# pydata/sparse

Measured on AMD Instinct MI355X. Metric: GCXS x dense SpMM throughput (GFLOP/s), higher is better.
Workload: dtype f32; 1 GPU; GCXS(CSR) 1000000x10000 @ 0.01 (100000000 nnz, int32 idx) in 1 nnz-balanced row block(s) x dense 10000x128 fp32; world_size=1, rows_rank0=1000000, idx_dtype=int32, parallelism=row-block x1, mul_add=fma, nan_warning=deferred, prewarm_products=40, default_settings=NAN_WARNING="sync" (verdict read inside every product), kernel=spmm_tiled (cached block stream)

## Files before the change

sparse_amd/_kernels.py:

```python
import os

import numpy as np
import torch

from . import _ffi
from ._device import code_of, np_dtype, ptr, require_hip, stream_ptr, torch_dtype


def dot_dtype(dt1, dt2):
    return (np.zeros((), dtype=np_dtype(dt1)) * np.zeros((), dtype=np_dtype(dt2))).dtype


_COMPLEX_CODE = {torch.complex64: _ffi.C64, torch.complex128: _ffi.C128}


def product_code(dt):
    dt = torch_dtype(dt)
    code = _COMPLEX_CODE.get(dt)
    return code_of(dt) if code is None else code


def _as_reals(t):
    return torch.view_as_real(t).reshape(-1) if t.is_complex() else t

# ... 1896 lines not shown
    return finish(exclusive_scan(nblk), lambda bo, total, blocks: _ffi.call(
        "spamd_spmm_tiled_pack", vc, nnz, ptr(tk), ptr(vals), ptr(seg_start), ptr(bo), total, ptr(blocks), s))


TILED_BALANCE = True
TILED_BALANCE_MIN_NNZ = 1 << 20
TILED_BALANCE_SKEW = 1.6
TILED_BALANCE_CAPMUL = 2
TILED_BALANCE_STATS = {}


def _balanced_tiled_layout(vals, ind, ptr_, M, Kd, dtype, nnz, defer_check, dev, s):
    rg, kb, gpb, epb, slack, direct_max, _ = tiled_params(dtype)
    ntiles = -(-Kd // kb)
    ic, vc = code_of(ind.dtype), code_of(_tiled_layout_dtype(dtype))
    mean_group = nnz * rg / max(M, 1)
    cap = 32
    while cap < TILED_BALANCE_CAPMUL * mean_group:
        cap *= 2
    stats = torch.empty(8, dtype=torch.int64, device=dev)
    _ffi.call("spamd_spmm_tiled_map_stats", ic, M, Kd, cap, ptr(ptr_), None, None, ptr(stats), s)
    st = stats.tolist()
    skew = st[6] / max(mean_group, 1.0)
    TILED_BALANCE_STATS.update(cap=cap, class_rows=st[:6], natural_max_group=st[6], skew=skew, balanced=False)
    if skew <= TILED_BALANCE_SKEW:
        return None
    keys = torch.empty(M, dtype=torch.int64, device=dev)
    rows = torch.empty(M, dtype=torch.int32, device=dev)
    _ffi.call("spamd_spmm_tiled_map_stats", ic, M, Kd, cap, ptr(ptr_), ptr(keys), ptr(rows), ptr(stats), s)
    st = stats.tolist()
    TILED_BALANCE_STATS.update(class_rows=st[:6])
    counts = _harr64(st[:6])
    groups = int(_ffi.lib().spamd_spmm_tiled_map_groups(counts))
    nseg = groups * ntiles
    upper = -(-nnz // epb) + nseg
    if groups <= 0 or upper >= 2 ** 31:
        return None
    keys, rows = sort_key_value(keys, rows, max(Kd, 1))
    rowmap = torch.empty(groups * rg + 16, dtype=torch.int32, device=dev)
    gload = torch.empty(groups + 1, dtype=torch.int64, device=dev)
    _ffi.call("spamd_spmm_tiled_map_build", ic, M, cap, ptr(ptr_), ptr(rows), counts, ptr(rowmap), ptr(gload), s)
    vstart = exclusive_scan(gload)
    blocks = torch.empty((upper + slack) * 16, dtype=torch.int32, device=dev)
    blk_off = torch.empty(groups * (ntiles + 1), dtype=torch.int32, device=dev)
    state = torch.empty(1, dtype=torch.int64, device=dev)
    _ffi.call("spamd_spmm_tiled_inspect_mapped", vc, ic, M, Kd, groups, ptr(vals), ptr(ind), ptr(ptr_), ptr(rowmap), ptr(vstart),
              ptr(state), ptr(blk_off), ptr(blocks), s)
    TILED_BALANCE_STATS.update(balanced=True, groups=groups)
    lay = TiledLayout(blocks, blk_off, dtype, nnz / epb / max(nseg, 1) + 0.5, group_ends=True, pending=state if defer_check else None,
                      rowmap=rowmap, groups=groups)
    if not defer_check and int(state[0]) != 0:
        return None
    return lay


def csc_tiled_layout(a_data, a_indices, a_indptr, M, Kd, dtype=None):
    dev = require_hip(a_data, a_indices, a_indptr)
    if dtype is None:
        dtype = a_data.dtype if a_data.dtype in TILED_DTYPES else torch.float32
    dtype = torch_dtype(dtype)
    rg, kb, gpb, epb, slack, direct_max, _ = tiled_params(dtype)
    nnz = int(a_data.numel())
    ntiles = -(-Kd // kb)
    groups = -(-(-(-M // rg)) // gpb) * gpb
    nseg = groups * ntiles
    upper = -(-nnz // epb) + nseg
    if ntiles > direct_max or upper >= 2 ** 31 or groups == 0 or not TILED_ONE_PASS_INSPECTOR:
        return None
    if not index_dtype_ok(a_indices) or a_indices.dtype != a_indptr.dtype:
        a_indices, a_indptr = a_indices.to(torch.int64), a_indptr.to(torch.int64)
    vals = a_data.to(dtype).contiguous()
    if dtype == torch.int32:
        vals = vals.view(torch.float32)
    blocks = torch.empty((upper + slack) * 16, dtype=torch.int32, device=dev)
    blk_off = torch.empty(groups * (ntiles + 1), dtype=torch.int32, device=dev)
    split = torch.empty(int(_ffi.lib().spamd_spmm_tiled_inspect_csc_ws(M, Kd)), dtype=torch.int32, device=dev)
    state = torch.empty(1, dtype=torch.int64, device=dev)
    _ffi.call("spamd_spmm_tiled_inspect_csc", code_of(_tiled_layout_dtype(dtype)), code_of(a_indices.dtype), M, Kd, ptr(vals),
              ptr(a_indices.contiguous()), ptr(a_indptr.contiguous()), ptr(split), ptr(state), ptr(blk_off), ptr(blocks),
              stream_ptr(dev))
    return TiledLayout(blocks, blk_off, dtype, nnz / epb / max(nseg, 1) + 0.5, group_ends=True, pending=state)


def dot_csr_ndarray_tiled(layout, out_shape, Kd, b, out=None, exact=False):
    blocks, blk_off, dtype = layout
    M, N = int(out_shape[0]), int(b.shape[1])
    Nout = int(out_shape[1])
    panel = 64 if dtype == torch.float64 else 128
    if N % panel or not (N - panel < Nout <= N):
        raise ValueError(f"tiled executor: B has {N} columns (whole {panel}-column panels expected), result {Nout}")
    last_cols = (Nout - (N - panel)) % panel
    dev = require_hip(blocks, blk_off, b)
    if b.dtype != dtype:
        raise TypeError(f"tiled layout holds {dtype} values, B is {b.dtype}")
    b = b.contiguous()
    if out is None:
        out = torch.empty((M, Nout), dtype=dtype, device=dev)
    lists = max(int(blk_off.numel()) - 1, 1)
    mean_blocks = getattr(layout, "mean_blocks", None) or (int(blocks.numel()) // 16) / lists
    hint = min(64, max(6, int(1.5 * mean_blocks) + 3))
    if _TOUCH_OVERRIDE:
        hint = _TOUCH_OVERRIDE
    ends = _ffi.TILED_GROUP_ENDS if getattr(layout, "group_ends", False) else 0
    ints = _ffi.TILED_INT32 if dtype == torch.int32 else 0
    flags = (_ffi.EXACT_MULADD if exact and not ints else 0) | ends | ints | (hint << 8) | (last_cols << 16)
    rowmap = getattr(layout, "rowmap", None)
    if rowmap is not None:
        _ffi.call("spamd_spmm_tiled_mapped", code_of(_tiled_layout_dtype(dtype)), M, int(layout.groups), Kd, N, ptr(blocks), ptr(blk_off),
                  ptr(rowmap), ptr(b), N, ptr(out), Nout, flags, stream_ptr(dev))
    else:
        _ffi.call("spamd_spmm_tiled", code_of(_tiled_layout_dtype(dtype)), M, Kd, N, ptr(blocks), ptr(blk_off), ptr(b), N, ptr(out), Nout,
                  flags, stream_ptr(dev))
    pending = getattr(layout, "pending", None)
    if pending is not None:
        layout.pending = None
        words = pending.tolist()
        mean = getattr(layout, "skew_mean", None)
        if mean and len(words) >= 8 and words[7] > TILED_BALANCE_SKEW * max(mean, 1.0):
            layout.rebalance = True
        if int(words[0]) != 0:
            raise UnsortedColumns("tiled layout built from rows with unsorted column indices")
    return out
```

sparse_amd/csrc/spmm_tiled.hip:

```cpp
#include "common.h"
#include "spmm_tiled_asm.inc"
#include <stdlib.h>
#include <mutex>
#include <set>

namespace spamd {

constexpr int TL_RG = TL_ASM_RG;
constexpr int TL_WAVES = TL_ASM_WAVES;
#ifndef SPAMD_TL_EXPERIMENTAL
static_assert(TL_RG == 35 && TL_WAVES == 16, "experimental tiled-SpMM geometry: build with -DSPAMD_TL_EXPERIMENTAL");
#endif
constexpr int TL_KB = TL_ASM_KB;
constexpr int TL_NBUF = 2;
__host__ __device__ constexpr int tl_d0(int lc, int lr) { return ((lc >> 1) << 11) | ((lc & 1) << 9) | (2 + 2 * lr); }
constexpr int TL_BLOCK_INTS = 16;

template <typename T>
struct TlFmt;
template <>
struct TlFmt<float> {
  static constexpr int EPB = 8, PANEL = 128;
  __device__ static void put(int* stream, int64_t entry, int d0, float v) {
    int* b = stream + (entry / EPB) * TL_BLOCK_INTS + (entry % EPB) * 2;
    typedef int int2v __attribute__((ext_vector_type(2)));
    int2v e;
    e.x = d0;
    e.y = __builtin_bit_cast(int, v);
    *reinterpret_cast<int2v*>(b) = e;
  }
};
template <>
struct TlFmt<double> {
  static constexpr int EPB = 5, PANEL = 64;
  __device__ static void put(int* stream, int64_t entry, int d0, double v) {
    int* b = stream + (entry / EPB) * TL_BLOCK_INTS;
    const int slot = (int)(entry % EPB);
    const long long bits = __builtin_bit_cast(long long, v);
    b[slot] = d0;
    if (slot == 0) b[5] = 0;
    *reinterpret_cast<long long*>(b + 6 + 2 * slot) = bits;
  }
};
typedef int tl_srd_t __attribute__((ext_vector_type(4)));
constexpr int TL_TILE = TL_KB * 512;
constexpr int TL_LDS = TL_NBUF * TL_TILE;
constexpr int TL_DMA_PER_TILE = TL_TILE / 16 / (TL_WAVES * 64);
static_assert(TL_LDS <= 160 * 1024 && TL_KB % (2 * TL_WAVES) == 0 && TL_DMA_PER_TILE == TL_ASM_DMA_PER_TILE,
              "tile geometry is baked into gen_tiled_asm.py");
constexpr int TL_SLACK_BLOCKS = 68;

#define GRID_STRIDE(i, n)                                                          \
  for (int64_t i = (int64_t)blockIdx.x * blockDim.x + threadIdx.x; i < (n);        \
       i += (int64_t)gridDim.x * blockDim.x)

__global__ void __launch_bounds__(256) tl_keys_kernel(const int64_t* __restrict__ rc_keys, int64_t nnz, int64_t K,
                                                      int64_t ntiles, int64_t* __restrict__ out) {
  GRID_STRIDE(i, nnz) {
    const int64_t k = rc_keys[i];
    const int64_t row = k / K, col = k - row * K;
    const int64_t g = row / TL_RG, lr = row - g * TL_RG, t = col / TL_KB, lc = col - t * TL_KB;
    out[i] = ((g * ntiles + t) * TL_RG + lr) * TL_KB + lc;
  }
}

__global__ void __launch_bounds__(256) tl_seg_start_kernel(const int64_t* __restrict__ keys, int64_t nnz,
                                                           int64_t nseg, int64_t* __restrict__ seg_start) {
  GRID_STRIDE(i, nnz + 1) {
    const int64_t hi = i < nnz ? keys[i] / (TL_RG * TL_KB) : nseg;
    const int64_t lo = i > 0 ? keys[i - 1] / (TL_RG * TL_KB) + 1 : 0;
    for (int64_t s = lo; s <= hi; ++s) seg_start[s] = i;
  }
}

__global__ void __launch_bounds__(256) tl_blocks_kernel(const int64_t* __restrict__ seg_start, int64_t nseg, int epb,
                                                        int64_t* __restrict__ nblk) {
  GRID_STRIDE(s, nseg + 1) {
    nblk[s] = s < nseg ? (seg_start[s + 1] - seg_start[s] + epb - 1) / epb : 0;
  }
}

template <typename T>
__global__ void __launch_bounds__(256) tl_pack_kernel(const int64_t* __restrict__ keys, const T* __restrict__ vals,
                                                      int64_t nnz, const int64_t* __restrict__ seg_start,
                                                      const int64_t* __restrict__ blk_off, int* __restrict__ stream) {
// ... 201 lines not shown
  const int gtotal = wtot[0] + wtot[1] + wtot[2] + wtot[3];
  const int my_off = woff + x - nb;
  const int64_t goff = tl_group_first_block(e0, g, ntiles, EPB);
  const int64_t gnext = tl_group_first_block(e1, g + 1, ntiles, EPB);
  if (tid < ntiles) loff[tid] = my_off;
  __syncthreads();
  if (tid < ntiles) blk_off[g * (ntiles + 1) + tid] = (int)(goff + my_off);
  if (tid == 0) blk_off[g * (ntiles + 1) + ntiles] = (int)(goff + gtotal);
  for (int64_t i = (goff + gtotal) * TL_BLOCK_INTS + tid; i < gnext * TL_BLOCK_INTS; i += 256) stream[i] = 0;
  if (group_bad) {
    for (int64_t i = goff * TL_BLOCK_INTS + tid; i < (goff + gtotal) * TL_BLOCK_INTS; i += 256) stream[i] = 0;
    return;
  }
  auto fill_one = [&](int lr, int64_t ra, int64_t e, unsigned c, T v) {
    const int t = (int)(c / (unsigned)TL_KB);
    const int lc = (int)(c - (unsigned)t * (unsigned)TL_KB);
    const int64_t dst = (goff + loff[t]) * EPB + before[lr * ntiles + t] + ((int)(e - (MAPPED ? ra : e0)) - runstart[lr * ntiles + t]);
    TlFmt<T>::put(stream, dst, tl_d0(lc, lr), v);
  };
#pragma unroll
  for (int i = 0; i < RPW; ++i) {
    const int lr = wv + 4 * i;
    if (lr >= TL_RG) break;
    const int64_t ra = rsab[2 * (lr)], rb = rsab[2 * (lr) + 1];
#pragma unroll
    for (int p = 0; p < TL_PRE; ++p) {
      const int64_t e = ra + lane + 64 * p;
      if (e < rb) fill_one(lr, ra, e, cpre[i][p], vpre[i][p]);
    }
    for (int64_t e = ra + lane + 64 * TL_PRE; e < rb; e += 64) fill_one(lr, ra, e, (unsigned)indices[e], vals[e]);
  }
  if (tid < ntiles) {
    const int64_t first = (goff + my_off) * EPB;
    for (int i = cnt_t; i < nb * EPB; ++i) TlFmt<T>::put(stream, first + i, 0, T(0));
  }
}

__device__ __forceinline__ void tl_dma16(unsigned lds_base, const void* src) {
  asm volatile("s_mov_b32 m0, %0\n\ts_nop 0\n\tglobal_load_lds_dwordx4 %1, off"
               :
               : "s"(lds_base), "v"(src)
               : "memory", "m0");
}

template <int MODE>
__device__ __forceinline__ void tl_phases(const int* stream, int t0, int te, int o0, int o1, int o2, int offreg, int obase,
                                          int ntiles, int nfull, int toff, int mask, unsigned m0wave,
                                          unsigned row_step, int voff, tl_srd_t srd, unsigned& soff) {
  const int lane = threadIdx.x & 63;
  const unsigned blo = (unsigned)((uintptr_t)stream & 0xffffffffu), bhi = (unsigned)((uintptr_t)stream >> 32);
  const int lane8 = lane * 8;
#define TL_PHASES_OPERANDS                                                                                        \
  [soff] "+s"(soff)                                                                                               \
  : [blo] "s"(blo), [bhi] "s"(bhi), [t0] "s"(t0), [te] "s"(te), [o0] "s"(o0), [o1] "s"(o1), [o2] "s"(o2),         \
    [obase] "s"(obase), [ntiles] "s"(ntiles), [nfull] "s"(nfull), [m0wave] "s"(m0wave), [step] "s"(row_step),      \
    [toff] "v"(toff), [lane8] "v"(lane8), [mask] "v"(mask), [offreg] "v"(offreg), [voff] "v"(voff), [srd] "s"(srd)  \
  : "memory", "m0", "scc", "vcc", TL_CLOB_SGPR, TL_CLOB_TMP, TL_CLOB_ACC
  if (MODE == 6)
    asm volatile(TL_ASM_PHASES_I32 : TL_PHASES_OPERANDS);
  else if (MODE == 4)
    asm volatile(TL_ASM_PHASES_F64 : TL_PHASES_OPERANDS);
  else if (MODE == 5)
    asm volatile(TL_ASM_PHASES_F64_EXACT : TL_PHASES_OPERANDS);
  else if (MODE == 3)
    asm volatile(TL_ASM_PHASES_EXACT : TL_PHASES_OPERANDS);
  else if (MODE == 1)
    asm volatile(TL_ASM_PHASES_NOFMA : TL_PHASES_OPERANDS);
  else if (MODE == 2)
    asm volatile(TL_ASM_PHASES_NOLDS : TL_PHASES_OPERANDS);
  else
    asm volatile(TL_ASM_PHASES : TL_PHASES_OPERANDS);
#undef TL_PHASES_OPERANDS
}

__device__ __forceinline__ void tl_block_map(unsigned L, int npanels, int nblocks, int& bx, int& by) {
  const unsigned pin = npanels > 1 ? 2u : 1u;
  const unsigned per_chunk = (unsigned)((nblocks + 7) / 8) * 8u * pin;
  const unsigned chunk = L / per_chunk, l = L % per_chunk;
  const unsigned seq = l >> 3;
  by = uniform((int)(chunk * pin + seq % pin));
  bx = uniform((int)((seq / pin) * 8u + (l & 7u)));
}

template <int DBG, int MODE, typename T>
__global__ void __launch_bounds__(TL_WAVES * 64) __attribute__((amdgpu_num_vgpr(TL_ASM_COMP)))
spmm_tiled_kernel(int64_t M, int64_t K, int ntiles, int touch_lines, const int* __restrict__ stream,
                  const int* __restrict__ blk_off, const T* __restrict__ b, int64_t ldb,
                  T* __restrict__ out, int64_t ldo, int last_cols, int npanels, int nblocks, const int* __restrict__ rowmap) {
  constexpr int PANEL = TlFmt<T>::PANEL;
  constexpr int CPL = PANEL / 64;
  extern __shared__ __attribute__((aligned(16))) char lds[];
  const int tid = threadIdx.x;
  const int lane = tid & 63;
  const int wv = uniform(tid >> 6);
  int bx, by;
  tl_block_map(blockIdx.x, npanels, nblocks, bx, by);
  if (bx >= nblocks || by >= npanels) return;
  const int g = bx * TL_WAVES + wv;
  b += (int64_t)by * PANEL;
  out += (int64_t)by * PANEL;

  asm volatile(TL_ASM_ZERO ::: "memory", TL_CLOB_ACC);

  const int nfull = DBG == 2 ? 0 : (int)(K / TL_KB);
  const unsigned row_step = (unsigned)((2 * TL_WAVES) * ldb * (int64_t)sizeof(T));
  const unsigned m0wave = (unsigned)wv * 2048u;
  const uint64_t bbase = (uint64_t)(uintptr_t)b;
  tl_srd_t srd;
  srd[0] = (int)(bbase & 0xffffffffu);
  srd[1] = (int)((bbase >> 32) & 0xffffu);
  srd[2] = (int)0xffffffffu;
  srd[3] = 0x00020000;
  const int voff = (int)((int64_t)(tid >> 5) * ldb * (int64_t)sizeof(T)) + (tid & 31) * 16;
  unsigned soff = 0;
  auto issue_partial = [&](int t) {
#pragma unroll
    for (int i = 0; i < TL_DMA_PER_TILE; ++i) {
      const int e = (i * (TL_WAVES * 64) + tid) * 16;
      int64_t r = (int64_t)t * TL_KB + (e >> 9);
      if (r >= K) r = K - 1;
      tl_dma16(((unsigned)(i * TL_WAVES + wv) * 2u + (unsigned)(t & 1)) * 1024u,
               reinterpret_cast<const char*>(b + r * ldb) + (e & 511));
    }
  };
  const bool has_partial = DBG != 2 && (int64_t)nfull * TL_KB < K;

  if (nfull > 0)
    asm volatile(TL_ASM_TILE0 : [soff] "+s"(soff) : [m0wave] "s"(m0wave), [step] "s"(row_step), [voff] "v"(voff), [srd] "s"(srd) : "memory", "m0", "scc", "vcc", "s89");
  else if (has_partial)
    issue_partial(0);
  asm volatile("s_waitcnt vmcnt(0)" ::: "memory");
  __syncthreads();

  const int* const myoff = blk_off + (int64_t)g * (ntiles + (touch_lines >> 16));
  touch_lines &= 0xffff;
  const int toff = (lane < touch_lines ? lane : touch_lines - 1) * 64;
  int t = 0;
  while (t < ntiles) {
    const int obase = t;
    const int q = obase + lane;
    int offreg = myoff[q < ntiles ? q : ntiles];
    asm volatile("" : "+v"(offreg));
    int te = obase + 61 < ntiles ? obase + 61 : ntiles;
    if (has_partial && t < nfull - 1 && nfull - 1 < te) te = nfull - 1;
    if (has_partial && t == nfull - 1) issue_partial(nfull);
    auto o = [&](int tt) { return wave_bcast(offreg, (tt < ntiles ? tt : ntiles) - obase); };
    const int o0 = o(t), o1 = o(t + 1), o2 = o(t + 2);
    if (t == 0) {
      const int n = o2 - o0, l = lane < n ? lane : 0;
      asm volatile("global_load_dword " TL_ASM_TOUCH ", %0, off" ::"v"(reinterpret_cast<const char*>(stream + (int64_t)o0 * 16) + l * 64)
                   : "memory", TL_ASM_TOUCH);
    }
    tl_phases<MODE>(stream, t, te, o0, o1, o2, offreg, obase, ntiles, nfull, toff, (int)0xfffffe00, m0wave, row_step, voff, srd, soff);
    t = te;
  }
  asm volatile("s_waitcnt vmcnt(0) lgkmcnt(0)" ::: "memory");

  const int64_t row0 = (int64_t)g * TL_RG;
  const int64_t left = M - row0;
  const int nvalid = left <= 0 ? 0 : (left < TL_RG ? (int)left : TL_RG);
  T* const obase_p = out + row0 * ldo + lane * CPL;
  const int64_t stride_bytes = ldo * (int64_t)sizeof(T);
  int bx2, by2;
  tl_block_map(blockIdx.x, npanels, nblocks, bx2, by2);
  const int ncols = (last_cols > 0 && by2 == npanels - 1) ? last_cols : PANEL;
  if (rowmap) {
    const int* const rm = rowmap + (int64_t)g * TL_RG;
    T* const base_p = out + lane * CPL;
    if (lane * CPL + CPL <= ncols)
      asm volatile(TL_ASM_STORE_PERM
                   :
                   : [lo] "v"((unsigned)((uintptr_t)base_p & 0xffffffffu)), [hi] "v"((unsigned)((uintptr_t)base_p >> 32)),
                     [stride] "s"((unsigned)stride_bytes), [rm] "s"(rm)
                   : "memory", "scc", TL_CLOB_SGPR, TL_CLOB_TMP, TL_CLOB_ACC);
    if constexpr (CPL == 2) {
      if (lane * CPL + 1 == ncols)
        asm volatile(TL_ASM_STORE1_PERM
                     :
                     : [lo] "v"((unsigned)((uintptr_t)base_p & 0xffffffffu)), [hi] "v"((unsigned)((uintptr_t)base_p >> 32)),
                       [stride] "s"((unsigned)stride_bytes), [rm] "s"(rm)
                     : "memory", "scc", TL_CLOB_SGPR, TL_CLOB_TMP);
    }
    return;
  }
  if (lane * CPL + CPL <= ncols)
    asm volatile(TL_ASM_STORE
                 :
                 : [lo] "v"((unsigned)((uintptr_t)obase_p & 0xffffffffu)), [hi] "v"((unsigned)((uintptr_t)obase_p >> 32)),
                   [stride] "s"(stride_bytes), [n] "s"(nvalid)
                 : "memory", "scc", "s36", TL_ASM_BASE, TL_ASM_TOUCH, TL_CLOB_ACC);
  if constexpr (CPL == 2) {
    if (lane * CPL + 1 == ncols)
      asm volatile(TL_ASM_STORE1
                   :
                   : [lo] "v"((unsigned)((uintptr_t)obase_p & 0xffffffffu)), [hi] "v"((unsigned)((uintptr_t)obase_p >> 32)),
                     [stride] "s"(stride_bytes), [n] "s"(nvalid)
                   : "memory", "scc", "s36", TL_ASM_BASE, TL_ASM_TOUCH);
  }
}

static int64_t tl_grid_groups(int64_t M) { return ceil_div(ceil_div(M, (int64_t)TL_RG), (int64_t)TL_WAVES) * TL_WAVES; }

}

using namespace spamd;

static int tl_epb(int val_dtype) { return val_dtype == SPAMD_F32 ? TlFmt<float>::EPB : (val_dtype == SPAMD_F64 ? TlFmt<double>::EPB : 0); }

extern "C" int spamd_spmm_tiled_params(int val_dtype, int* rows_per_group, int* tile_rows, int* groups_per_block,
                                       int* entries_per_block, int* slack_blocks, int* direct_max_tiles,
                                       int* panel_cols) {
  if (!tl_epb(val_dtype)) return SPAMD_ETYPE;
  if (direct_max_tiles) *direct_max_tiles = TL_DIRECT_MAX_TILES;
  if (rows_per_group) *rows_per_group = TL_RG;
  if (tile_rows) *tile_rows = TL_KB;
  if (groups_per_block) *groups_per_block = TL_WAVES;
  if (entries_per_block) *entries_per_block = tl_epb(val_dtype);
  if (slack_blocks) *slack_blocks = TL_SLACK_BLOCKS;
  if (panel_cols) *panel_cols = val_dtype == SPAMD_F32 ? TlFmt<float>::PANEL : TlFmt<double>::PANEL;
  return 0;
}

static unsigned tl_blocks_for(int64_t n) {
  int64_t blocks = ceil_div(n, (int64_t)256);
  if (blocks > 8192) blocks = 8192;
  if (blocks < 1) blocks = 1;
  return (unsigned)blocks;
}

extern "C" int spamd_spmm_tiled_keys(int64_t nnz, const int64_t* rowcol_keys, int64_t K, int64_t* tiled_keys,
                                     void* stream) {
  if (nnz < 0 || K <= 0) return SPAMD_EINVAL;
  if (nnz == 0) return 0;
  hipLaunchKernelGGL(tl_keys_kernel, dim3(tl_blocks_for(nnz)), dim3(256), 0, (hipStream_t)stream, rowcol_keys, nnz, K,
                     ceil_div(K, (int64_t)TL_KB), tiled_keys);
  return launch_status();
}

extern "C" int spamd_spmm_tiled_lists(int val_dtype, int64_t nnz, const int64_t* tiled_keys_sorted, int64_t M, int64_t K,
                                      int64_t* seg_start, int64_t* nblk, void* stream) {
  if (nnz < 0 || M < 0 || K <= 0) return SPAMD_EINVAL;
  if (!tl_epb(val_dtype)) return SPAMD_ETYPE;
  const int64_t nseg = tl_grid_groups(M) * ceil_div(K, (int64_t)TL_KB);
  hipLaunchKernelGGL(tl_seg_start_kernel, dim3(tl_blocks_for(nnz + 1)), dim3(256), 0, (hipStream_t)stream,
                     tiled_keys_sorted, nnz, nseg, seg_start);
  hipLaunchKernelGGL(tl_blocks_kernel, dim3(tl_blocks_for(nseg + 1)), dim3(256), 0, (hipStream_t)stream, seg_start,
                     nseg, tl_epb(val_dtype), nblk);
  return launch_status();
}

static int tl_clear_blocks(int64_t total_blocks, int* blocks, hipStream_t s) {
  return (int)hipMemsetAsync(blocks, 0, (size_t)(total_blocks + TL_SLACK_BLOCKS) * TL_BLOCK_INTS * sizeof(int), s);
}

extern "C" int spamd_spmm_tiled_pack(int val_dtype, int64_t nnz, const int64_t* tiled_keys_sorted, const void* vals_sorted,
                                     const int64_t* seg_start, const int64_t* blk_off, int64_t total_blocks,
                                     int* blocks, void* stream) {
  if (nnz < 0 || total_blocks < 0) return SPAMD_EINVAL;
  if (!tl_epb(val_dtype)) return SPAMD_ETYPE;
  int rc = tl_clear_blocks(total_blocks, blocks, (hipStream_t)stream);
  if (rc) return rc;
  if (nnz == 0) return 0;
  if (val_dtype == SPAMD_F32)
    hipLaunchKernelGGL(tl_pack_kernel<float>, dim3(tl_blocks_for(nnz)), dim3(256), 0, (hipStream_t)stream, tiled_keys_sorted,
                       (const float*)vals_sorted, nnz, seg_start, blk_off, blocks);
  else
    hipLaunchKernelGGL(tl_pack_kernel<double>, dim3(tl_blocks_for(nnz)), dim3(256), 0, (hipStream_t)stream, tiled_keys_sorted,
                       (const double*)vals_sorted, nnz, seg_start, blk_off, blocks);
  return launch_status();
}

extern "C" int spamd_spmm_tiled_count(int val_dtype, int idx_dtype, int64_t M, int64_t K, const void* a_indices,
                                      const void* a_indptr, int64_t* nblk, int* flags, void* stream) {
  if (M < 0 || K <= 0) return SPAMD_EINVAL;
  if (!tl_epb(val_dtype)) return SPAMD_ETYPE;
  const int64_t ntiles = ceil_div(K, (int64_t)TL_KB);
  if (ntiles > TL_DIRECT_MAX_TILES) return SPAMD_EINVAL;
  const int64_t groups = tl_grid_groups(M);
  hipError_t e = hipMemsetAsync(flags, 0, sizeof(int), (hipStream_t)stream);
  if (e != hipSuccess) return (int)e;
// ... 756 lines not shown
      for (int q = c; q < nb * EPB; ++q) TlFmt<T>::put(stream, first + q, 0, T(0));
    }
    __syncthreads();
  }
}

template <typename I, typename T>
static int tl_launch_inspect_csc(int64_t M, int64_t K, int64_t ntiles, const T* a_data, const I* a_indices, const I* a_indptr,
                                 int* ws, unsigned long long* state, int* blk_off, int* blocks, hipStream_t s) {
  const int64_t groups = tl_grid_groups(M);
  const int64_t nblocks = groups / TL_WAVES;
  if (nblocks >= ((int64_t)1 << 31)) return SPAMD_EINVAL;
  const bool hist = groups <= TL_CSC_HIST_GROUPS;
  int* const split = ws;
  int* const cnt = split + (nblocks + 1) * K;
  int* const rel = cnt + TL_CSC_HIST_PARTS * groups * ntiles;
  const int64_t words = ((nblocks + 1) * K + TL_CSC_HIST_PARTS * groups * ntiles + groups * (ntiles + 1) + 1) & ~(int64_t)1;
  unsigned long long* const look = reinterpret_cast<unsigned long long*>(ws + words);
  long long* const e0 = reinterpret_cast<long long*>(look) + groups;
  const int64_t owgs = ceil_div(groups, (int64_t)64);
  const int nlook = (int)(owgs + 2);
  static_assert(TL_WAVES >= 3, "groups (a multiple of TL_WAVES) >= ceil(groups / 64) + 2");
  if (!hist) {
    const unsigned sgrid = (unsigned)std::min<int64_t>(K, (int64_t)256 * 64);
    hipLaunchKernelGGL((tl_csc_split_kernel<I>), dim3(sgrid), dim3(256), 0, s, M, K, nblocks, a_indices, a_indptr, split, state, look, nlook);
  }
  const dim3 grid((unsigned)nblocks, (unsigned)ceil_div(ntiles, (int64_t)TL_CSC_TC));
  if (hist) {
    auto hk = &tl_csc_hist_kernel<I>;
    const int lds = (int)((groups + 1) / 2 * sizeof(int));
    if (lds > 48 * 1024) {
      hipError_t e = hipFuncSetAttribute(reinterpret_cast<const void*>(hk), hipFuncAttributeMaxDynamicSharedMemorySize, lds);
      if (e != hipSuccess) return (int)e;
    }
    hipLaunchKernelGGL(hk, dim3((unsigned)ntiles, TL_CSC_HIST_PARTS), dim3(1024), lds, s, M, K, (int)ntiles, groups, nblocks,
                       a_indices, a_indptr, cnt, split, state, look, nlook);
  } else {
    hipLaunchKernelGGL((tl_csc_count_kernel<I>), grid, dim3(256), 0, s, K, (int)ntiles, nblocks, groups, a_indices, a_indptr, (const int*)split,
                       (const unsigned long long*)state, cnt);
  }
  if (hist)
    hipLaunchKernelGGL((tl_csc_offsets_kernel<TlFmt<T>::EPB, TL_CSC_HIST_PARTS>), dim3((unsigned)owgs), dim3(64), 0, s,
                       groups, (int)ntiles, (const int*)cnt, (const unsigned long long*)state, rel, look, e0);
  else
    hipLaunchKernelGGL((tl_csc_offsets_kernel<TlFmt<T>::EPB, 1>), dim3((unsigned)owgs), dim3(64), 0, s,
                       groups, (int)ntiles, (const int*)cnt, (const unsigned long long*)state, rel, look, e0);
  const int64_t fgrid = 8 * ceil_div(nblocks, (int64_t)8) * ceil_div(ntiles, (int64_t)TL_CSC_TC);
  if (fgrid >= ((int64_t)1 << 31)) return SPAMD_EINVAL;
  hipLaunchKernelGGL((tl_csc_fill_kernel<I, T>), dim3((unsigned)fgrid), dim3(256), 0, s, K, (int)ntiles, a_data, a_indices,
                     a_indptr, (const int*)split, (const unsigned long long*)state, (const int*)rel, (const long long*)e0, nblocks,
                     blk_off, blocks);
  return launch_status();
}

extern "C" int64_t spamd_spmm_tiled_inspect_csc_ws(int64_t M, int64_t K) {
  if (M < 0 || K <= 0) return -1;
  const int64_t ntiles = ceil_div(K, (int64_t)TL_KB), groups = tl_grid_groups(M), nblocks = groups / TL_WAVES;
  return (nblocks + 1) * K + TL_CSC_HIST_PARTS * groups * ntiles + groups * (ntiles + 1) + 2 + 2 * (2 * groups + 1) + 16;
}

extern "C" int spamd_spmm_tiled_inspect_csc(int val_dtype, int idx_dtype, int64_t M, int64_t K, const void* a_data,
                                            const void* a_indices, const void* a_indptr, int* ws, void* state, int* blk_off,
                                            int* blocks, void* stream) {
  if (M < 0 || K <= 0) return SPAMD_EINVAL;
  if (!tl_epb(val_dtype)) return SPAMD_ETYPE;
  if ((uintptr_t)ws % 8) return SPAMD_EINVAL;
  const int64_t ntiles = ceil_div(K, (int64_t)TL_KB);
  if (ntiles > TL_DIRECT_MAX_TILES) return SPAMD_EINVAL;
  hipError_t e = hipMemsetAsync(state, 0, sizeof(unsigned long long), (hipStream_t)stream);
  if (e != hipSuccess) return (int)e;
  if (tl_grid_groups(M) == 0) return 0;
  SPAMD_DISPATCH_IDX(idx_dtype, I, {
    if (val_dtype == SPAMD_F32)
      return tl_launch_inspect_csc<I, float>(M, K, ntiles, (const float*)a_data, (const I*)a_indices, (const I*)a_indptr, ws,
                                             (unsigned long long*)state, blk_off, blocks, (hipStream_t)stream);
    return tl_launch_inspect_csc<I, double>(M, K, ntiles, (const double*)a_data, (const I*)a_indices, (const I*)a_indptr, ws,
                                            (unsigned long long*)state, blk_off, blocks, (hipStream_t)stream);
  })
  return SPAMD_ETYPE;
}

static int tl_set_lds_once(const void* kern) { return set_max_dynamic_lds(kern, TL_LDS); }

template <typename T, typename KERN>
static int tl_launch(KERN kern, int64_t M, int64_t K, int64_t N, const int* blocks, const int* blk_off, const T* b,
                     int64_t ldb, T* out, int64_t ldo, int touch_lines, bool group_ends, int last_cols, hipStream_t s,
                     const int* rowmap = nullptr, int64_t map_groups = 0) {
  if (int rc = tl_set_lds_once(reinterpret_cast<const void*>(kern))) return rc;
  const int64_t blocks_n = (rowmap ? map_groups : tl_grid_groups(M)) / TL_WAVES;
  const int64_t npanels = N / TlFmt<T>::PANEL;
  const int64_t grid = ceil_div(blocks_n, (int64_t)8) * 8 * (npanels > 1 ? ceil_div(npanels, (int64_t)2) * 2 : 1);
  if (grid >= ((int64_t)1 << 31) || blocks_n >= ((int64_t)1 << 31)) return SPAMD_EINVAL;
  hipLaunchKernelGGL(kern, dim3((unsigned)grid), dim3(TL_WAVES * 64), TL_LDS, s, M, K,
                     (int)ceil_div(K, (int64_t)TL_KB), touch_lines | (group_ends ? 1 << 16 : 0), blocks, blk_off, b, ldb, out, ldo,
                     last_cols, (int)npanels, (int)blocks_n, rowmap);
  return launch_status();
}

static int tl_product(int val_dtype, int64_t M, int64_t K, int64_t N, const int* blocks, const int* blk_off, const void* b,
                      int64_t ldb, void* out, int64_t ldo, unsigned flags, void* stream, const int* rowmap, int64_t map_groups);

extern "C" int spamd_spmm_tiled(int val_dtype, int64_t M, int64_t K, int64_t N, const int* blocks, const int* blk_off,
                                const void* b, int64_t ldb, void* out, int64_t ldo, unsigned flags, void* stream) {
  return tl_product(val_dtype, M, K, N, blocks, blk_off, b, ldb, out, ldo, flags, stream, nullptr, 0);
}

extern "C" int spamd_spmm_tiled_mapped(int val_dtype, int64_t M, int64_t groups, int64_t K, int64_t N, const int* blocks,
                                       const int* blk_off, const int* rowmap, const void* b, int64_t ldb, void* out, int64_t ldo,
                                       unsigned flags, void* stream) {
  if (!rowmap || groups <= 0 || groups % TL_WAVES) return SPAMD_EINVAL;
  if (ldo * (val_dtype == SPAMD_F32 ? 4 : 8) >= ((int64_t)1 << 32)) return SPAMD_EINVAL;
  return tl_product(val_dtype, M, K, N, blocks, blk_off, b, ldb, out, ldo, flags | SPAMD_TILED_GROUP_ENDS, stream, rowmap, groups);
}

static int tl_product(int val_dtype, int64_t M, int64_t K, int64_t N, const int* blocks, const int* blk_off, const void* b,
                      int64_t ldb, void* out, int64_t ldo, unsigned flags, void* stream, const int* rowmap, int64_t map_groups) {
  if (!tl_epb(val_dtype)) return SPAMD_ETYPE;
  const int panel = val_dtype == SPAMD_F32 ? TlFmt<float>::PANEL : TlFmt<double>::PANEL;
  const int esz = val_dtype == SPAMD_F32 ? 4 : 8;
  if (M < 0 || K <= 0 || N <= 0 || N % panel != 0 || N / panel > 65535 || K / TL_KB >= ((int64_t)1 << 30)) return SPAMD_EINVAL;
  if (M == 0) return 0;
  if (((uintptr_t)b % 16) || ((ldb * esz) % 16) || ((uintptr_t)out % esz) || ((uintptr_t)blocks % 64))
    return SPAMD_EINVAL;
  if ((K + 2 * TL_KB) * ldb * esz >= ((int64_t)1 << 32)) return SPAMD_EINVAL;
  hipStream_t s = (hipStream_t)stream;
  const bool exact = (flags & SPAMD_EXACT_MULADD) != 0;
  const bool ends = (flags & SPAMD_TILED_GROUP_ENDS) != 0;
  const bool i32 = (flags & SPAMD_TILED_INT32) != 0;
  if (i32 && val_dtype != SPAMD_F32) return SPAMD_EINVAL;
  const int last_cols = (int)((flags >> 16) & 0xffu);
  if (last_cols > panel) return SPAMD_EINVAL;
  if (ldo < N - panel + (last_cols ? last_cols : panel)) return SPAMD_EINVAL;
  int touch = (int)((flags >> 8) & 0xffu);
  if (touch == 0) touch = 12;
  if (touch > 64) touch = 64;
  if (val_dtype == SPAMD_F64) {
    const double* bb = (const double*)b;
    double* oo = (double*)out;
    return exact ? tl_launch<double>(&spmm_tiled_kernel<0, 5, double>, M, K, N, blocks, blk_off, bb, ldb, oo, ldo, touch, ends, last_cols, s, rowmap, map_groups)
                 : tl_launch<double>(&spmm_tiled_kernel<0, 4, double>, M, K, N, blocks, blk_off, bb, ldb, oo, ldo, touch, ends, last_cols, s, rowmap, map_groups);
  }
  const float* bb = (const float*)b;
  float* oo = (float*)out;
#ifdef SPAMD_TUNING
  const char* dbg_env = getenv("SPAMD_TILED_DBG");
  const int dbg = dbg_env ? atoi(dbg_env) : 0;
  if (dbg == 2) return tl_launch<float>(&spmm_tiled_kernel<2, 0, float>, M, K, N, blocks, blk_off, bb, ldb, oo, ldo, touch, ends, last_cols, s, rowmap, map_groups);
  if (dbg == 5) return tl_launch<float>(&spmm_tiled_kernel<0, 1, float>, M, K, N, blocks, blk_off, bb, ldb, oo, ldo, touch, ends, last_cols, s, rowmap, map_groups);
  if (dbg == 6) return tl_launch<float>(&spmm_tiled_kernel<0, 2, float>, M, K, N, blocks, blk_off, bb, ldb, oo, ldo, touch, ends, last_cols, s, rowmap, map_groups);
  if (dbg == 7) return tl_launch<float>(&spmm_tiled_kernel<2, 2, float>, M, K, N, blocks, blk_off, bb, ldb, oo, ldo, touch, ends, last_cols, s, rowmap, map_groups);
#endif
  if (i32) return tl_launch<float>(&spmm_tiled_kernel<0, 6, float>, M, K, N, blocks, blk_off, bb, ldb, oo, ldo, touch, ends, last_cols, s, rowmap, map_groups);
  return exact ? tl_launch<float>(&spmm_tiled_kernel<0, 3, float>, M, K, N, blocks, blk_off, bb, ldb, oo, ldo, touch, ends, last_cols, s, rowmap, map_groups)
               : tl_launch<float>(&spmm_tiled_kernel<0, 0, float>, M, K, N, blocks, blk_off, bb, ldb, oo, ldo, touch, ends, last_cols, s, rowmap, map_groups);
}
```

Before: 30260 GFLOP/s.

## Make tiled SpMM kernel persistent, prefetching next block's first tile before storing

Converts the tiled SpMM kernel into a persistent kernel. With a single panel and no rowmap, the grid is limited to roughly one workgroup per CU, and each workgroup loops over logical blocks. Before storing the current block's accumulators, it starts the next block's B-tile DMA and offset load, so launch and prologue latency overlap with the epilogue. It also prefetches the next chunk's offsets inside the tile loop and passes kernel args by struct read from the kernarg segment to save registers. The risks are reduced occupancy and latency hiding, plus more scalar reloads.

```diff
diff --git a/sparse_amd/_kernels.py b/sparse_amd/_kernels.py
--- a/sparse_amd/_kernels.py
+++ b/sparse_amd/_kernels.py
@@ -2002,8 +2002,11 @@
     return TiledLayout(blocks, blk_off, dtype, nnz / epb / max(nseg, 1) + 0.5, group_ends=True, pending=state)
 
 
-def dot_csr_ndarray_tiled(layout, out_shape, Kd, b, out=None, exact=False):
+def dot_csr_ndarray_tiled(layout, out_shape, Kd, b, out=None, exact=False, resident=0):
     blocks, blk_off, dtype = layout
+    resident = int(resident)
+    if resident < 0 or resident % 8 or resident > 127 * 8:
+        raise ValueError(f"tiled executor: resident = {resident} (a multiple of 8 in [0, 1016] expected)")
     M, N = int(out_shape[0]), int(b.shape[1])
     Nout = int(out_shape[1])
     panel = 64 if dtype == torch.float64 else 128
@@ -2023,7 +2026,7 @@
         hint = _TOUCH_OVERRIDE
     ends = _ffi.TILED_GROUP_ENDS if getattr(layout, "group_ends", False) else 0
     ints = _ffi.TILED_INT32 if dtype == torch.int32 else 0
-    flags = (_ffi.EXACT_MULADD if exact and not ints else 0) | ends | ints | (hint << 8) | (last_cols << 16)
+    flags = (_ffi.EXACT_MULADD if exact and not ints else 0) | ends | ints | (hint << 8) | (last_cols << 16) | ((resident // 8) << 24)
     rowmap = getattr(layout, "rowmap", None)
     if rowmap is not None:
         _ffi.call("spamd_spmm_tiled_mapped", code_of(_tiled_layout_dtype(dtype)), M, int(layout.groups), Kd, N, ptr(blocks), ptr(blk_off),
diff --git a/sparse_amd/csrc/spmm_tiled.hip b/sparse_amd/csrc/spmm_tiled.hip
--- a/sparse_amd/csrc/spmm_tiled.hip
+++ b/sparse_amd/csrc/spmm_tiled.hip
@@ -1,6 +1,7 @@
 #include "common.h"
 #include "spmm_tiled_asm.inc"
 #include <stdlib.h>
+#include <atomic>
 #include <mutex>
 #include <set>
 
@@ -368,120 +369,247 @@
   bx = uniform((int)((seq / pin) * 8u + (l & 7u)));
 }
 
+template <typename T>
+struct TlArgs {
+  int64_t M, K;
+  const int* stream;
+  const int* blk_off;
+  const T* b;
+  int64_t ldb;
+  T* out;
+  int64_t ldo;
+  const int* rowmap;
+  int ntiles, touch_lines, last_cols, npanels, nblocks;
+  int total;
+  int grid;
+#ifdef SPAMD_TUNING
+  unsigned long long* stamps;
+#endif
+};
+
+#ifdef SPAMD_TUNING
+constexpr int TL_STAMPS = 12;
+static unsigned long long* tl_timeline_buf = nullptr;
+#define TL_STAMP(L, slot)                                                                      \
+  do {  \
+    unsigned long long* const st_ = tl_args<T>()->stamps;                                      \
+    if (st_ && uniform(tl_park(tid) >> 6) == 0) st_[(int64_t)(L) * TL_STAMPS + (slot)] = wall_clock64(); \
+  } while (0)
+#else
+#define TL_STAMP(L, slot) \
+  do {                    \
+  } while (0)
+#endif
+
+template <typename T>
+__device__ __forceinline__ const __attribute__((address_space(4))) TlArgs<T>* tl_args() {
+  auto p = (const __attribute__((address_space(4))) TlArgs<T>*)__builtin_amdgcn_kernarg_segment_ptr();
+  asm volatile("" : "+s"(p));
+  return p;
+}
+
+__device__ __forceinline__ int tl_park(int x) {
+  asm volatile("" : "+v"(x));
+  return x;
+}
+__device__ __forceinline__ int tl_fresh(int x) {
+  asm volatile("" : "+s"(x));
+  return x;
+}
+
+__device__ __forceinline__ int tl_next_block(int L, int grid, int total, int npanels, int nblocks) {
+  while (L < total) {
+    int bx, by;
+    tl_block_map((unsigned)L, npanels, nblocks, bx, by);
+    if (bx < nblocks && by < npanels) break;
+    L += grid;
+  }
+  return L;
+}
+
 template <int DBG, int MODE, typename T>
 __global__ void __launch_bounds__(TL_WAVES * 64) __attribute__((amdgpu_num_vgpr(TL_ASM_COMP)))
-spmm_tiled_kernel(int64_t M, int64_t K, int ntiles, int touch_lines, const int* __restrict__ stream,
-                  const int* __restrict__ blk_off, const T* __restrict__ b, int64_t ldb,
-                  T* __restrict__ out, int64_t ldo, int last_cols, int npanels, int nblocks, const int* __restrict__ rowmap) {
+spmm_tiled_kernel(const TlArgs<T> a) {
   constexpr int PANEL = TlFmt<T>::PANEL;
   constexpr int CPL = PANEL / 64;
   extern __shared__ __attribute__((aligned(16))) char lds[];
   const int tid = threadIdx.x;
   const int lane = tid & 63;
   const int wv = uniform(tid >> 6);
-  int bx, by;
-  tl_block_map(blockIdx.x, npanels, nblocks, bx, by);
-  if (bx >= nblocks || by >= npanels) return;
-  const int g = bx * TL_WAVES + wv;
-  b += (int64_t)by * PANEL;
-  out += (int64_t)by * PANEL;
+  auto block_of = [&](int L, int& g, int& by) {
+    const auto ap = tl_args<T>();
+    int bx;
+    tl_block_map((unsigned)L, ap->npanels, ap->nblocks, bx, by);
+    g = bx * TL_WAVES + wv;
+  };
+  auto next_block = [&](int L) {
+    const auto ap = tl_args<T>();
+    return tl_next_block(L, ap->grid, ap->total, ap->npanels, ap->nblocks);
+  };
+  int Lv = tl_park(next_block((int)blockIdx.x));
+  if (uniform(Lv) >= tl_args<T>()->total) return;
 
   asm volatile(TL_ASM_ZERO ::: "memory", TL_CLOB_ACC);
 
-  const int nfull = DBG == 2 ? 0 : (int)(K / TL_KB);
-  const unsigned row_step = (unsigned)((2 * TL_WAVES) * ldb * (int64_t)sizeof(T));
+  const int ntiles = a.ntiles;
+  const int* const stream = a.stream;
+  const int nfull = DBG == 2 ? 0 : (int)(a.K / TL_KB);
+  const unsigned row_step = (unsigned)((2 * TL_WAVES) * a.ldb * (int64_t)sizeof(T));
   const unsigned m0wave = (unsigned)wv * 2048u;
-  const uint64_t bbase = (uint64_t)(uintptr_t)b;
   tl_srd_t srd;
-  srd[0] = (int)(bbase & 0xffffffffu);
-  srd[1] = (int)((bbase >> 32) & 0xffffu);
   srd[2] = (int)0xffffffffu;
   srd[3] = 0x00020000;
-  const int voff = (int)((int64_t)(tid >> 5) * ldb * (int64_t)sizeof(T)) + (tid & 31) * 16;
+  const int voff = (int)((int64_t)(tid >> 5) * a.ldb * (int64_t)sizeof(T)) + (tid & 31) * 16;
   unsigned soff = 0;
   auto issue_partial = [&](int t) {
-#pragma unroll
+    const auto ap = tl_args<T>();
+    const int64_t K = ap->K, ldb = ap->ldb;
+    const int tidp = tl_park(tid);
+    const char* const b = reinterpret_cast<const char*>((uintptr_t)(((uint64_t)(unsigned)srd[1] << 32) | (unsigned)srd[0]));
+#pragma nounroll
     for (int i = 0; i < TL_DMA_PER_TILE; ++i) {
-      const int e = (i * (TL_WAVES * 64) + tid) * 16;
+      const int e = (i * (TL_WAVES * 64) + tidp) * 16;
       int64_t r = (int64_t)t * TL_KB + (e >> 9);
       if (r >= K) r = K - 1;
       tl_dma16(((unsigned)(i * TL_WAVES + wv) * 2u + (unsigned)(t & 1)) * 1024u,
-               reinterpret_cast<const char*>(b + r * ldb) + (e & 511));
+               b + (unsigned)(r * ldb * (int64_t)sizeof(T)) + (e & 511));
     }
   };
-  const bool has_partial = DBG != 2 && (int64_t)nfull * TL_KB < K;
-
-  if (nfull > 0)
-    asm volatile(TL_ASM_TILE0 : [soff] "+s"(soff) : [m0wave] "s"(m0wave), [step] "s"(row_step), [voff] "v"(voff), [srd] "s"(srd) : "memory", "m0", "scc", "vcc", "s89");
-  else if (has_partial)
-    issue_partial(0);
-  asm volatile("s_waitcnt vmcnt(0)" ::: "memory");
-  __syncthreads();
-
-  const int* const myoff = blk_off + (int64_t)g * (ntiles + (touch_lines >> 16));
-  touch_lines &= 0xffff;
-  const int toff = (lane < touch_lines ? lane : touch_lines - 1) * 64;
-  int t = 0;
-  while (t < ntiles) {
-    const int obase = t;
-    const int q = obase + lane;
-    int offreg = myoff[q < ntiles ? q : ntiles];
-    asm volatile("" : "+v"(offreg));
-    int te = obase + 61 < ntiles ? obase + 61 : ntiles;
-    if (has_partial && t < nfull - 1 && nfull - 1 < te) te = nfull - 1;
-    if (has_partial && t == nfull - 1) issue_partial(nfull);
-    auto o = [&](int tt) { return wave_bcast(offreg, (tt < ntiles ? tt : ntiles) - obase); };
-    const int o0 = o(t), o1 = o(t + 1), o2 = o(t + 2);
-    if (t == 0) {
-      const int n = o2 - o0, l = lane < n ? lane : 0;
-      asm volatile("global_load_dword " TL_ASM_TOUCH ", %0, off" ::"v"(reinterpret_cast<const char*>(stream + (int64_t)o0 * 16) + l * 64)
-                   : "memory", TL_ASM_TOUCH);
-    }
-    tl_phases<MODE>(stream, t, te, o0, o1, o2, offreg, obase, ntiles, nfull, toff, (int)0xfffffe00, m0wave, row_step, voff, srd, soff);
-    t = te;
-  }
-  asm volatile("s_waitcnt vmcnt(0) lgkmcnt(0)" ::: "memory");
-
-  const int64_t row0 = (int64_t)g * TL_RG;
-  const int64_t left = M - row0;
-  const int nvalid = left <= 0 ? 0 : (left < TL_RG ? (int)left : TL_RG);
-  T* const obase_p = out + row0 * ldo + lane * CPL;
-  const int64_t stride_bytes = ldo * (int64_t)sizeof(T);
-  int bx2, by2;
-  tl_block_map(blockIdx.x, npanels, nblocks, bx2, by2);
-  const int ncols = (last_cols > 0 && by2 == npanels - 1) ? last_cols : PANEL;
-  if (rowmap) {
-    const int* const rm = rowmap + (int64_t)g * TL_RG;
-    T* const base_p = out + lane * CPL;
-    if (lane * CPL + CPL <= ncols)
-      asm volatile(TL_ASM_STORE_PERM
-                   :
-                   : [lo] "v"((unsigned)((uintptr_t)base_p & 0xffffffffu)), [hi] "v"((unsigned)((uintptr_t)base_p >> 32)),
-                     [stride] "s"((unsigned)stride_bytes), [rm] "s"(rm)
-                   : "memory", "scc", TL_CLOB_SGPR, TL_CLOB_TMP, TL_CLOB_ACC);
-    if constexpr (CPL == 2) {
-      if (lane * CPL + 1 == ncols)
-        asm volatile(TL_ASM_STORE1_PERM
-                     :
-                     : [lo] "v"((unsigned)((uintptr_t)base_p & 0xffffffffu)), [hi] "v"((unsigned)((uintptr_t)base_p >> 32)),
-                       [stride] "s"((unsigned)stride_bytes), [rm] "s"(rm)
-                     : "memory", "scc", TL_CLOB_SGPR, TL_CLOB_TMP);
-    }
-    return;
-  }
-  if (lane * CPL + CPL <= ncols)
-    asm volatile(TL_ASM_STORE
-                 :
-                 : [lo] "v"((unsigned)((uintptr_t)obase_p & 0xffffffffu)), [hi] "v"((unsigned)((uintptr_t)obase_p >> 32)),
-                   [stride] "s"(stride_bytes), [n] "s"(nvalid)
-                 : "memory", "scc", "s36", TL_ASM_BASE, TL_ASM_TOUCH, TL_CLOB_ACC);
-  if constexpr (CPL == 2) {
-    if (lane * CPL + 1 == ncols)
-      asm volatile(TL_ASM_STORE1
-                   :
-                   : [lo] "v"((unsigned)((uintptr_t)obase_p & 0xffffffffu)), [hi] "v"((unsigned)((uintptr_t)obase_p >> 32)),
-                     [stride] "s"(stride_bytes), [n] "s"(nvalid)
-                   : "memory", "scc", "s36", TL_ASM_BASE, TL_ASM_TOUCH);
+  auto has_partial = [&] { return DBG != 2 && tl_fresh(nfull) < ntiles; };
+
+  int toff;
+  {
+    const int touch_lines = a.touch_lines & 0xffff;
+    toff = (lane < touch_lines ? lane : touch_lines - 1) * 64;
+  }
+  auto offsets_of = [&](int g) {
+    const auto ap = tl_args<T>();
+    return ap->blk_off + (int64_t)tl_park(g) * (ap->ntiles + (ap->touch_lines >> 16));
+  };
+
+  auto start_block = [&](int L) {
+    int g, by;
+    block_of(L, g, by);
+    const uint64_t bbase = (uint64_t)(uintptr_t)(tl_args<T>()->b + (int64_t)by * PANEL);
+    srd[0] = (int)(bbase & 0xffffffffu);
+    srd[1] = (int)((bbase >> 32) & 0xffffu);
+    soff = 0;
+    if (tl_fresh(nfull) > 0)
+      asm volatile(TL_ASM_TILE0 : [soff] "+s"(soff) : [m0wave] "s"(m0wave), [step] "s"(row_step), [voff] "v"(voff), [srd] "s"(srd) : "memory", "m0", "scc", "vcc", "s89");
+    else if (has_partial())
+      issue_partial(0);
+    const int lanep = tl_park(lane);
+    return offsets_of(g)[lanep < ntiles ? lanep : ntiles];
+  };
+
+  TL_STAMP(uniform(Lv), 0);
+  int offreg = start_block(uniform(Lv));
+  for (;;) {
+    asm volatile("s_waitcnt vmcnt(0)" ::: "memory");
+    __syncthreads();
+    {
+#ifdef SPAMD_TUNING
+      int chunk = 0;
+      TL_STAMP(uniform(Lv), 1);
+#endif
+      int g, by;
+      block_of(uniform(Lv), g, by);
+      const int* const myoff = offsets_of(g);
+      int t = 0;
+#pragma nounroll
+      while (t < ntiles) {
+        const int obase = t;
+        asm volatile("" : "+v"(offreg));
+        int te = obase + 61 < ntiles ? obase + 61 : ntiles;
+        if (has_partial() && t < nfull - 1 && nfull - 1 < te) te = nfull - 1;
+        int offnext = 0;
+        if (te < ntiles) {
+          const int q = te + lane;
+          offnext = myoff[q < ntiles ? q : ntiles];
+        }
+        if (has_partial() && t == nfull - 1) issue_partial(nfull);
+        auto o = [&](int tt) { return wave_bcast(offreg, (tt < ntiles ? tt : ntiles) - obase); };
+        const int o0 = o(t), o1 = o(t + 1), o2 = o(t + 2);
+        if (t == 0) {
+          const int n = o2 - o0, l = lane < n ? lane : 0;
+          asm volatile("global_load_dword " TL_ASM_TOUCH ", %0, off" ::"v"(reinterpret_cast<const char*>(stream + (int64_t)o0 * 16) + l * 64)
+                       : "memory", TL_ASM_TOUCH);
+        }
+#ifdef SPAMD_TUNING
+        TL_STAMP(uniform(Lv), 2 + (chunk < TL_STAMPS - 5 ? chunk : TL_STAMPS - 5));
+        ++chunk;
+#endif
+        tl_phases<MODE>(stream, t, te, o0, o1, o2, offreg, obase, ntiles, nfull, toff, (int)0xfffffe00, m0wave, row_step, voff, srd, soff);
+        t = te;
+        offreg = offnext;
+      }
+    }
+    asm volatile("s_waitcnt vmcnt(0) lgkmcnt(0)" ::: "memory");
+    Lv = tl_park(Lv);
+    const int L = uniform(Lv);
+    TL_STAMP(L, TL_STAMPS - 2);
+
+    const int Ln = next_block(L + tl_args<T>()->grid);
+    const bool more = Ln < tl_args<T>()->total;
+    if (more) {
+      __syncthreads();
+      offreg = start_block(Ln);
+    }
+
+    {
+      const auto ap = tl_args<T>();
+      const int lane = tl_park(tid) & 63;
+      int g, by;
+      block_of(L, g, by);
+      T* const out = ap->out + (int64_t)by * PANEL;
+      const int64_t ldo = ap->ldo;
+      const int64_t stride_bytes = ldo * (int64_t)sizeof(T);
+      const int last_cols = ap->last_cols;
+      const int ncols = (last_cols > 0 && by == ap->npanels - 1) ? last_cols : PANEL;
+      const int* const rowmap = ap->rowmap;
+      if (rowmap) {
+        const int* const rm = rowmap + (int64_t)g * TL_RG;
+        T* const base_p = out + lane * CPL;
+        if (lane * CPL + CPL <= ncols)
+          asm volatile(TL_ASM_STORE_PERM
+                       :
+                       : [lo] "v"((unsigned)((uintptr_t)base_p & 0xffffffffu)), [hi] "v"((unsigned)((uintptr_t)base_p >> 32)),
+                         [stride] "s"((unsigned)stride_bytes), [rm] "s"(rm)
+                       : "memory", "scc", TL_CLOB_SGPR, TL_CLOB_TMP, TL_CLOB_ACC);
+        if constexpr (CPL == 2) {
+          if (lane * CPL + 1 == ncols)
+            asm volatile(TL_ASM_STORE1_PERM
+                         :
+                         : [lo] "v"((unsigned)((uintptr_t)base_p & 0xffffffffu)), [hi] "v"((unsigned)((uintptr_t)base_p >> 32)),
+                           [stride] "s"((unsigned)stride_bytes), [rm] "s"(rm)
+                         : "memory", "scc", TL_CLOB_SGPR, TL_CLOB_TMP);
+        }
+      } else {
+        const int64_t row0 = (int64_t)g * TL_RG;
+        const int64_t left = ap->M - row0;
+        const int nvalid = left <= 0 ? 0 : (left < TL_RG ? (int)left : TL_RG);
+        T* const obase_p = out + row0 * ldo + lane * CPL;
+        if (lane * CPL + CPL <= ncols)
+          asm volatile(TL_ASM_STORE
+                       :
+                       : [lo] "v"((unsigned)((uintptr_t)obase_p & 0xffffffffu)), [hi] "v"((unsigned)((uintptr_t)obase_p >> 32)),
+                         [stride] "s"(stride_bytes), [n] "s"(nvalid)
+                       : "memory", "scc", "s36", TL_ASM_BASE, TL_ASM_TOUCH, TL_CLOB_ACC);
+        if constexpr (CPL == 2) {
+          if (lane * CPL + 1 == ncols)
+            asm volatile(TL_ASM_STORE1
+                         :
+                         : [lo] "v"((unsigned)((uintptr_t)obase_p & 0xffffffffu)), [hi] "v"((unsigned)((uintptr_t)obase_p >> 32)),
+                           [stride] "s"(stride_bytes), [n] "s"(nvalid)
+                         : "memory", "scc", "s36", TL_ASM_BASE, TL_ASM_TOUCH);
+        }
+      }
+    }
+    TL_STAMP(L, TL_STAMPS - 1);
+    if (!more) return;
+    asm volatile(TL_ASM_ZERO ::: "memory", TL_CLOB_ACC);
+    TL_STAMP(Ln, 0);
+    Lv = tl_park(Ln);
   }
 }
 
@@ -1404,20 +1532,61 @@
 
 static int tl_set_lds_once(const void* kern) { return set_max_dynamic_lds(kern, TL_LDS); }
 
+static int tl_device_cus(int* cus) {
+  constexpr int MAX_DEV = 64;
+  static std::atomic<int> cached[MAX_DEV];
+  int dev = 0;
+  if (hipError_t e = hipGetDevice(&dev); e != hipSuccess) return (int)e;
+  int n = dev >= 0 && dev < MAX_DEV ? cached[dev].load(std::memory_order_relaxed) : 0;
+  if (n <= 0) {
+    if (hipError_t e = hipDeviceGetAttribute(&n, hipDeviceAttributeMultiprocessorCount, dev); e != hipSuccess) return (int)e;
+    if (n <= 0) return SPAMD_EINVAL;
+    if (dev >= 0 && dev < MAX_DEV) cached[dev].store(n, std::memory_order_relaxed);
+  }
+  *cus = n;
+  return 0;
+}
+
 template <typename T, typename KERN>
 static int tl_launch(KERN kern, int64_t M, int64_t K, int64_t N, const int* blocks, const int* blk_off, const T* b,
                      int64_t ldb, T* out, int64_t ldo, int touch_lines, bool group_ends, int last_cols, hipStream_t s,
-                     const int* rowmap = nullptr, int64_t map_groups = 0) {
+                     const int* rowmap, int64_t map_groups, int resident) {
   if (int rc = tl_set_lds_once(reinterpret_cast<const void*>(kern))) return rc;
   const int64_t blocks_n = (rowmap ? map_groups : tl_grid_groups(M)) / TL_WAVES;
   const int64_t npanels = N / TlFmt<T>::PANEL;
-  const int64_t grid = ceil_div(blocks_n, (int64_t)8) * 8 * (npanels > 1 ? ceil_div(npanels, (int64_t)2) * 2 : 1);
-  if (grid >= ((int64_t)1 << 31) || blocks_n >= ((int64_t)1 << 31)) return SPAMD_EINVAL;
-  hipLaunchKernelGGL(kern, dim3((unsigned)grid), dim3(TL_WAVES * 64), TL_LDS, s, M, K,
-                     (int)ceil_div(K, (int64_t)TL_KB), touch_lines | (group_ends ? 1 << 16 : 0), blocks, blk_off, b, ldb, out, ldo,
-                     last_cols, (int)npanels, (int)blocks_n, rowmap);
+  const int64_t total = ceil_div(blocks_n, (int64_t)8) * 8 * (npanels > 1 ? ceil_div(npanels, (int64_t)2) * 2 : 1);
+  if (total >= ((int64_t)1 << 31) - 2048 || blocks_n >= ((int64_t)1 << 31)) return SPAMD_EINVAL;
+  int64_t res = (int64_t)resident * 8;
+  if (res == 0) {
+    if (rowmap || npanels > 1) {
+      res = total;
+    } else {
+      int cus = 0;
+      if (int rc = tl_device_cus(&cus)) return rc;
+      res = ceil_div((int64_t)cus, (int64_t)8) * 8;
+    }
+  }
+#ifdef SPAMD_TUNING
+  if (getenv("SPAMD_TILED_ONE_BLOCK")) res = total;
+#endif
+  const int64_t grid = total < res ? total : res;
+  TlArgs<T> args{};
+  args.M = M, args.K = K, args.stream = blocks, args.blk_off = blk_off, args.b = b, args.ldb = ldb, args.out = out, args.ldo = ldo;
+  args.rowmap = rowmap, args.ntiles = (int)ceil_div(K, (int64_t)TL_KB), args.touch_lines = touch_lines | (group_ends ? 1 << 16 : 0);
+  args.last_cols = last_cols, args.npanels = (int)npanels, args.nblocks = (int)blocks_n, args.total = (int)total, args.grid = (int)grid;
+#ifdef SPAMD_TUNING
+  args.stamps = tl_timeline_buf;
+#endif
+  hipLaunchKernelGGL(kern, dim3((unsigned)grid), dim3(TL_WAVES * 64), TL_LDS, s, args);
   return launch_status();
 }
+
+#ifdef SPAMD_TUNING
+extern "C" int spamd_spmm_tiled_timeline(void* buf) {
+  tl_timeline_buf = (unsigned long long*)buf;
+  return TL_STAMPS;
+}
+#endif
 
 static int tl_product(int val_dtype, int64_t M, int64_t K, int64_t N, const int* blocks, const int* blk_off, const void* b,
                       int64_t ldb, void* out, int64_t ldo, unsigned flags, void* stream, const int* rowmap, int64_t map_groups);
@@ -1456,23 +1625,24 @@
   int touch = (int)((flags >> 8) & 0xffu);
   if (touch == 0) touch = 12;
   if (touch > 64) touch = 64;
+  const int resident = (int)((flags >> 24) & 0x7fu);
   if (val_dtype == SPAMD_F64) {
     const double* bb = (const double*)b;
     double* oo = (double*)out;
-    return exact ? tl_launch<double>(&spmm_tiled_kernel<0, 5, double>, M, K, N, blocks, blk_off, bb, ldb, oo, ldo, touch, ends, last_cols, s, rowmap, map_groups)
-                 : tl_launch<double>(&spmm_tiled_kernel<0, 4, double>, M, K, N, blocks, blk_off, bb, ldb, oo, ldo, touch, ends, last_cols, s, rowmap, map_groups);
+    return exact ? tl_launch<double>(&spmm_tiled_kernel<0, 5, double>, M, K, N, blocks, blk_off, bb, ldb, oo, ldo, touch, ends, last_cols, s, rowmap, map_groups, resident)
+                 : tl_launch<double>(&spmm_tiled_kernel<0, 4, double>, M, K, N, blocks, blk_off, bb, ldb, oo, ldo, touch, ends, last_cols, s, rowmap, map_groups, resident);
   }
   const float* bb = (const float*)b;
   float* oo = (float*)out;
 #ifdef SPAMD_TUNING
   const char* dbg_env = getenv("SPAMD_TILED_DBG");
   const int dbg = dbg_env ? atoi(dbg_env) : 0;
-  if (dbg == 2) return tl_launch<float>(&spmm_tiled_kernel<2, 0, float>, M, K, N, blocks, blk_off, bb, ldb, oo, ldo, touch, ends, last_cols, s, rowmap, map_groups);
-  if (dbg == 5) return tl_launch<float>(&spmm_tiled_kernel<0, 1, float>, M, K, N, blocks, blk_off, bb, ldb, oo, ldo, touch, ends, last_cols, s, rowmap, map_groups);
-  if (dbg == 6) return tl_launch<float>(&spmm_tiled_kernel<0, 2, float>, M, K, N, blocks, blk_off, bb, ldb, oo, ldo, touch, ends, last_cols, s, rowmap, map_groups);
-  if (dbg == 7) return tl_launch<float>(&spmm_tiled_kernel<2, 2, float>, M, K, N, blocks, blk_off, bb, ldb, oo, ldo, touch, ends, last_cols, s, rowmap, map_groups);
-#endif
-  if (i32) return tl_launch<float>(&spmm_tiled_kernel<0, 6, float>, M, K, N, blocks, blk_off, bb, ldb, oo, ldo, touch, ends, last_cols, s, rowmap, map_groups);
-  return exact ? tl_launch<float>(&spmm_tiled_kernel<0, 3, float>, M, K, N, blocks, blk_off, bb, ldb, oo, ldo, touch, ends, last_cols, s, rowmap, map_groups)
-               : tl_launch<float>(&spmm_tiled_kernel<0, 0, float>, M, K, N, blocks, blk_off, bb, ldb, oo, ldo, touch, ends, last_cols, s, rowmap, map_groups);
-}
+  if (dbg == 2) return tl_launch<float>(&spmm_tiled_kernel<2, 0, float>, M, K, N, blocks, blk_off, bb, ldb, oo, ldo, touch, ends, last_cols, s, rowmap, map_groups, resident);
+  if (dbg == 5) return tl_launch<float>(&spmm_tiled_kernel<0, 1, float>, M, K, N, blocks, blk_off, bb, ldb, oo, ldo, touch, ends, last_cols, s, rowmap, map_groups, resident);
+  if (dbg == 6) return tl_launch<float>(&spmm_tiled_kernel<0, 2, float>, M, K, N, blocks, blk_off, bb, ldb, oo, ldo, touch, ends, last_cols, s, rowmap, map_groups, resident);
+  if (dbg == 7) return tl_launch<float>(&spmm_tiled_kernel<2, 2, float>, M, K, N, blocks, blk_off, bb, ldb, oo, ldo, touch, ends, last_cols, s, rowmap, map_groups, resident);
+#endif
+  if (i32) return tl_launch<float>(&spmm_tiled_kernel<0, 6, float>, M, K, N, blocks, blk_off, bb, ldb, oo, ldo, touch, ends, last_cols, s, rowmap, map_groups, resident);
+  return exact ? tl_launch<float>(&spmm_tiled_kernel<0, 3, float>, M, K, N, blocks, blk_off, bb, ldb, oo, ldo, touch, ends, last_cols, s, rowmap, map_groups, resident)
+               : tl_launch<float>(&spmm_tiled_kernel<0, 0, float>, M, K, N, blocks, blk_off, bb, ldb, oo, ldo, touch, ends, last_cols, s, rowmap, map_groups, resident);
+}
```

New measurement: 30270 GFLOP/s, median of 2. No clear change (+0.0%).
